# annikabrundyn/driving-dirty

Measured on AMD Instinct MI355X. Metric: 6-view scenes/sec fwd+bwd, roadmap model bs=32, higher is better.
Workload: dtype f32

## Files before the change

driving-dirty_amd/csrc/conv3x3.hip:

```cpp
#include <stdlib.h>

#include "dd_common.h"

namespace {

constexpr int EPI_BIAS_RELU_BITS = 5;
constexpr int EPI_RELU_BITS = 6;
constexpr int EPI_BIAS_STATS = 7;
constexpr int EPI_RELU_MASK_AFF = 8;
constexpr int EPI_RELU_BITS_W1 = 9;


template <int CIN, int S>
struct StripCfg {
  static constexpr int PXB = CIN * 4;
  static constexpr int CHUNKS = CIN / 4;
  static constexpr int NPX = 32 * S + 2;
  static constexpr int SLOTB = NPX * PXB;
  static constexpr int NCH = NPX * CHUNKS;
  static constexpr int NLOAD = (NCH + 63) / 64;
  static constexpr int SPILLB = (NLOAD * 64 - NCH) * 16;
  static constexpr int WAVEB = 3 * SLOTB + SPILLB;
  static constexpr int KGROUPS = (CIN == 32) ? 36 : 5;
  static constexpr int WFLOATS = KGROUPS * 64 * 4;
};

template <int CIN>
__device__ __forceinline__ int swz(int q) {
  return CIN == 32 ? ((q >> 1) & 7) : 0;
}

template <int CIN, int S>
__device__ __forceinline__ void load_row(const float* __restrict__ img, int H, int W, int iy, int gx0, int lane,
                                         f32x4 (&r)[StripCfg<CIN, S>::NLOAD]) {
  using C = StripCfg<CIN, S>;
  const bool rowok = (iy >= 0) && (iy < H);
  const __amdgpu_buffer_rsrc_t rs = dd_rsrc(img + (long)(rowok ? iy : 0) * W * CIN, rowok ? W * C::PXB : 0);
#pragma unroll
  for (int i = 0; i < C::NLOAD; ++i) {
    const int c = lane + 64 * i;
    const int q = c / C::CHUNKS, ch = c % C::CHUNKS;
    const int off = (c < C::NCH) ? ((gx0 + q) * C::PXB + ch * 16) : -16;
    r[i] = dd_bload4<DD_AUX_NT>(rs, off);
  }
}

template <int CIN, int S>
__device__ __forceinline__ void load_row_img(const float* __restrict__ img, int H, int W, int iy, int gx0, int lane,
                                             f32x4 (&r)[StripCfg<CIN, S>::NLOAD]) {
  using C = StripCfg<CIN, S>;
  const bool rowok = (iy >= 0) && (iy < H);
  const int so = rowok ? iy * W * C::PXB : 0;
  const __amdgpu_buffer_rsrc_t rs = dd_rsrc(img, rowok ? so + W * C::PXB : 0);
#pragma unroll
  for (int i = 0; i < C::NLOAD; ++i) {
    const int c = lane + 64 * i;
    const int q = c / C::CHUNKS, ch = c % C::CHUNKS;
    const int off = (c < C::NCH) ? ((gx0 + q) * C::PXB + ch * 16) : -16;
    r[i] = dd_bload4<DD_AUX_NT>(rs, off, so);
  }
}

template <int CIN, int S, bool SWZ>
__device__ __forceinline__ void store_row(char* slot, char* spill, int lane,
                                          const f32x4 (&r)[StripCfg<CIN, S>::NLOAD]) {
  using C = StripCfg<CIN, S>;
#pragma unroll
  for (int i = 0; i < C::NLOAD; ++i) {
    const int c = lane + 64 * i;
    const int q = c / C::CHUNKS, ch = c % C::CHUNKS;
    char* dst = slot + q * C::PXB + ((ch ^ (SWZ ? swz<CIN>(q) : 0)) << 4);
    if (64 * (i + 1) > C::NCH) dst = (c < C::NCH) ? dst : spill + (c - C::NCH) * 16;
    *(f32x4*)dst = r[i];
  }
}

template <int S, bool SWZ>
__device__ __forceinline__ void store_row_aff(char* slot, char* spill, int lane, const f32x4 (&r)[StripCfg<32, S>::NLOAD],
                                              bool rowok, int gx0, int W, f32x4 sc, f32x4 sh) {
  using C = StripCfg<32, S>;
#pragma unroll
  for (int i = 0; i < C::NLOAD; ++i) {
    const int c = lane + 64 * i;
    const int q = c / C::CHUNKS, ch = c % C::CHUNKS;
    char* dst = slot + q * C::PXB + ((ch ^ (SWZ ? swz<32>(q) : 0)) << 4);
    if (64 * (i + 1) > C::NCH) dst = (c < C::NCH) ? dst : spill + (c - C::NCH) * 16;
    const bool in = rowok && (gx0 + q >= 0) && (gx0 + q < W);
    f32x4 v = r[i];
    v.x = in ? fmaxf(v.x * sc.x + sh.x, 0.f) : 0.f;
    v.y = in ? fmaxf(v.y * sc.y + sh.y, 0.f) : 0.f;
    v.z = in ? fmaxf(v.z * sc.z + sh.z, 0.f) : 0.f;
    v.w = in ? fmaxf(v.w * sc.w + sh.w, 0.f) : 0.f;
    *(f32x4*)dst = v;
  }
}

template <int CIN, int S, int EPI, int WPB, bool AFF = false>
__global__ __launch_bounds__(WPB * 64) void conv_strip_fwd(const float* __restrict__ x, const float* __restrict__ wp,
                                                           const float* __restrict__ bias,
                                                           const float* __restrict__ msk, float* __restrict__ y,
                                                           unsigned* __restrict__ bits_out, int B, int H, int W, int Ho,
                                                           int Wo, int nstrips, const float* __restrict__ aff = nullptr,
                                                           float* __restrict__ stats = nullptr) {
  using C = StripCfg<CIN, S>;
  extern __shared__ __attribute__((aligned(16))) char smem[];
  const int tid = threadIdx.x;
  const int lane = tid & 63;
  const int wave = __builtin_amdgcn_readfirstlane(tid >> 6);
  {
    f32x4* wl4 = (f32x4*)smem;
    const f32x4* wg4 = (const f32x4*)wp;
    for (int i = tid; i < C::WFLOATS / 4; i += WPB * 64) wl4[i] = wg4[i];
  }
  __syncthreads();
  char* ring = smem + C::WFLOATS * 4 + wave * C::WAVEB;
  char* spill = ring + 3 * C::SLOTB;
  const char* wl = smem;
  const int h = lane >> 5, n = lane & 31;
  const float bv = (EPI == DD_EPI_BIAS || EPI == DD_EPI_BIAS_RELU || EPI == EPI_BIAS_RELU_BITS || EPI == EPI_BIAS_STATS) ? bias[n] : 0.f;
  f32x4 asc = {1.f, 1.f, 1.f, 1.f}, ash = {0.f, 0.f, 0.f, 0.f};
  if (AFF) {
    asc = *(const f32x4*)(aff + 4 * (lane & 7));
    ash = *(const f32x4*)(aff + 32 + 4 * (lane & 7));
  }
  const float msc = (EPI == EPI_RELU_MASK_AFF) ? aff[64 + n] : 1.f, msh = (EPI == EPI_RELU_MASK_AFF) ? aff[96 + n] : 0.f;
  float st_sum = 0.f, st_sq = 0.f;

  long idx, end;
  dd_range((long)B * nstrips * Ho, blockIdx.x * WPB + wave, gridDim.x * WPB, idx, end);
  while (idx < end) {
    const long col = idx / Ho;
    const int y0 = (int)(idx - col * Ho);
    const int y1 = (int)min((long)Ho, y0 + (end - idx));
    idx += y1 - y0;
    const int b = (int)(col / nstrips), x0 = (int)(col % nstrips) * 32;
    const float* xb = x + (long)b * H * W * CIN;
    const int gx0 = S * x0 - 1;

#pragma unroll
    for (int d = 0; d < 3; ++d) {
      f32x4 t[C::NLOAD];
      const int iy = S * y0 - 1 + d;
      load_row<CIN, S>(xb, H, W, iy, gx0, lane, t);
      if constexpr (AFF) store_row_aff<S, true>(ring + ((iy + 1) % 3) * C::SLOTB, spill, lane, t, iy >= 0 && iy < H, gx0, W, asc, ash);
      else store_row<CIN, S, true>(ring + ((iy + 1) % 3) * C::SLOTB, spill, lane, t);
    }

    for (int yy = y0; yy < y1; ++yy) {
      f32x4 pre[S][C::NLOAD];
#pragma unroll
      for (int s = 0; s < S; ++s) load_row<CIN, S>(xb, H, W, S * yy + 2 + s, gx0, lane, pre[s]);

      const long orow = ((long)(b * Ho + yy) * Wo) * 32;
      float mreg[16];
      if (EPI == DD_EPI_RELU_MASK || EPI == EPI_RELU_MASK_AFF) {
        const __amdgpu_buffer_rsrc_t ms = dd_rsrc(msk + orow, Wo * 128);
#pragma unroll
        for (int r = 0; r < 16; ++r) mreg[r] = dd_bload1<DD_AUX_NT>(ms, ((x0 + dd_acc_row(r, lane)) * 32 + n) * 4);
      }
      if (EPI == EPI_RELU_BITS) {
        const __amdgpu_buffer_rsrc_t ms = dd_rsrc((const unsigned*)msk + (long)(b * Ho + yy) * Wo, Wo * 4);
#pragma unroll
        for (int r = 0; r < 16; ++r) mreg[r] = dd_bload1<DD_AUX_NT>(ms, (x0 + dd_acc_row(r, lane)) * 4);
      }
      __builtin_amdgcn_sched_barrier(0);

      f32x16 acc;
#pragma unroll
      for (int r = 0; r < 16; ++r) acc[r] = 0.f;

      if (CIN == 32) {
#pragma unroll
        for (int dy = 0; dy < 3; ++dy) {
          const char* rowb = ring + ((S * yy + dy) % 3) * C::SLOTB;
#pragma unroll
          for (int dx = 0; dx < 3; ++dx) {
            const int q = S * n + dx;
            const char* pa = rowb + q * 128;
            const int sw = swz<32>(q);
#pragma unroll
            for (int j = 0; j < 4; ++j) {
              const f32x4 a = *(const f32x4*)(pa + (((2 * j + h) ^ sw) << 4));
              const f32x4 w = *(const f32x4*)(wl + (((dy * 3 + dx) * 4 + j) * 64 + lane) * 16);
              acc = DD_MFMA(a.x, w.x, acc);
              acc = DD_MFMA(a.y, w.y, acc);
              acc = DD_MFMA(a.z, w.z, acc);
              acc = DD_MFMA(a.w, w.w, acc);
            }
          }
        }
      } else {
#pragma unroll
        for (int jp = 0; jp < 5; ++jp) {
          const int tap = min(2 * jp + h, 8);
          const int dy = tap / 3, dx = tap - 3 * dy;
          const char* rowb = ring + ((S * yy + dy) % 3) * C::SLOTB;
          const f32x4 a = *(const f32x4*)(rowb + (S * n + dx) * 16);
          const f32x4 w = *(const f32x4*)(wl + (jp * 64 + lane) * 16);
          acc = DD_MFMA(a.x, w.x, acc);
          acc = DD_MFMA(a.y, w.y, acc);
          acc = DD_MFMA(a.z, w.z, acc);
        }
      }

#pragma unroll
      for (int s = 0; s < S; ++s) {
        const int iy = S * yy + 2 + s;
        if constexpr (AFF) store_row_aff<S, true>(ring + ((iy + 1) % 3) * C::SLOTB, spill, lane, pre[s], iy >= 0 && iy < H, gx0, W, asc, ash);
        else store_row<CIN, S, true>(ring + ((iy + 1) % 3) * C::SLOTB, spill, lane, pre[s]);
      }

      const __amdgpu_buffer_rsrc_t ys = dd_rsrc(y + orow, Wo * 128);
      unsigned sign_word = 0;
#pragma unroll
      for (int r = 0; r < 16; ++r) {
        float v = acc[r];
        if (EPI == DD_EPI_BIAS || EPI == EPI_BIAS_STATS) v += bv;
        if (EPI == EPI_BIAS_STATS && x0 + dd_acc_row(r, lane) < Wo) {
          st_sum += v;
          st_sq += v * v;
        }
        if (EPI == DD_EPI_BIAS_RELU || EPI == EPI_BIAS_RELU_BITS) v = fmaxf(v + bv, 0.f);
        if (EPI == DD_EPI_RELU_MASK) v = (mreg[r] > 0.f) ? v : 0.f;
        if (EPI == EPI_RELU_MASK_AFF) v = (mreg[r] * msc + msh > 0.f) ? v : 0.f;
        if (EPI == EPI_RELU_BITS) v = ((__builtin_bit_cast(unsigned, mreg[r]) >> n) & 1u) ? v : 0.f;
        dd_bstore1<DD_AUX_NT>(ys, ((x0 + dd_acc_row(r, lane)) * 32 + n) * 4, v);
        if (EPI == EPI_BIAS_RELU_BITS) {
          const unsigned long long m = __ballot(v > 0.f);
          const int i0 = (r & 3) + 8 * (r >> 2);
          if (n == i0) sign_word = (unsigned)m;
          if (n == i0 + 4) sign_word = (unsigned)(m >> 32);
        }
      }
      if (EPI == EPI_BIAS_RELU_BITS) {
        const __amdgpu_buffer_rsrc_t bs = dd_rsrc(bits_out + (long)(b * Ho + yy) * Wo, Wo * 4);
        __builtin_amdgcn_raw_buffer_store_b32(sign_word, bs, (h == 0) ? (x0 + n) * 4 : -16, 0, 0);
      }
    }
  }
  if (EPI == EPI_BIAS_STATS) {
    const long gwl = ((long)(blockIdx.x * WPB + wave) * 64 + lane) * 2;
    stats[gwl] = st_sum;
    stats[gwl + 1] = st_sq;
  }
}

template <int WPB, int MASK>
__global__ __launch_bounds__(WPB * 64) void conv_s2_dgrad(const float* __restrict__ dy, const float* __restrict__ wp,
                                                          const float* __restrict__ msk, float* __restrict__ dx,
                                                          int B, int H, int W, int Ho, int Wo, int nstrips,
                                                          const float* __restrict__ aff = nullptr) {
  using C = StripCfg<32, 1>;
  extern __shared__ __attribute__((aligned(16))) char smem[];
  const int tid = threadIdx.x;
  const int lane = tid & 63;
  const int wave = __builtin_amdgcn_readfirstlane(tid >> 6);
  {
    f32x4* wl4 = (f32x4*)smem;
    const f32x4* wg4 = (const f32x4*)wp;
    for (int i = tid; i < C::WFLOATS / 4; i += WPB * 64) wl4[i] = wg4[i];
  }
  __syncthreads();
  const int nr = (H + 1) / 2;
  const float msc = (MASK == 3) ? aff[64 + (lane & 31)] : 1.f, msh = (MASK == 3) ? aff[96 + (lane & 31)] : 0.f;
  char* ring = smem + C::WFLOATS * 4 + wave * C::WAVEB;
  char* spill = ring + 3 * C::SLOTB;
  const char* wl = smem;
  const int h = lane >> 5, n = lane & 31;

  long idx, end;
  dd_range((long)B * nstrips * nr, blockIdx.x * WPB + wave, gridDim.x * WPB, idx, end);
  while (idx < end) {
    const long col = idx / nr;
    const int r0 = (int)(idx - col * nr);
    const int r1 = (int)min((long)nr, r0 + (end - idx));
    idx += r1 - r0;
    const int b = (int)(col / nstrips), s0 = (int)(col % nstrips) * 32;
    const float* dyb = dy + (long)b * Ho * Wo * 32;

#pragma unroll
    for (int d = 0; d < 2; ++d) {
      f32x4 t[C::NLOAD];
      load_row<32, 1>(dyb, Ho, Wo, r0 + d, s0, lane, t);
      store_row<32, 1, true>(ring + ((r0 + d) % 3) * C::SLOTB, spill, lane, t);
    }

    for (int r = r0; r < r1; ++r) {
      f32x4 pre[C::NLOAD];
      load_row<32, 1>(dyb, Ho, Wo, r + 2, s0, lane, pre);
      __builtin_amdgcn_sched_barrier(0);

      const char* row_r = ring + (r % 3) * C::SLOTB;
      const char* row_r1 = ring + ((r + 1) % 3) * C::SLOTB;
#define DD_TILE(PY, PX, NTAP, ...)                                                              \
  {                                                                                             \
    constexpr int taps[NTAP][3] = {__VA_ARGS__};                                                \
    const int yi = 2 * r + (PY);                                                                \
    const long orow = ((long)(b * H + min(yi, H - 1)) * W) * 32;                                \
    const int obytes = (yi < H) ? W * 128 : 0;                                                  \
    float mreg[16];                                                                             \
    if (MASK == 1 || MASK == 3) {                                                               \
      const __amdgpu_buffer_rsrc_t ms = dd_rsrc(msk + orow, obytes);                            \
      _Pragma("unroll") for (int rr = 0; rr < 16; ++rr)                                         \
        mreg[rr] = dd_bload1<DD_AUX_NT>(ms, ((2 * (s0 + dd_acc_row(rr, lane)) + (PX)) * 32 + n) * 4); \
      __builtin_amdgcn_sched_barrier(0);                                                        \
    }                                                                                           \
    if (MASK == 2) {                                                                            \
      const __amdgpu_buffer_rsrc_t ms = dd_rsrc((const unsigned*)msk + (long)(b * H + min(yi, H - 1)) * W, obytes / 32); \
      _Pragma("unroll") for (int rr = 0; rr < 16; ++rr)                                         \
        mreg[rr] = dd_bload1<DD_AUX_NT>(ms, (2 * (s0 + dd_acc_row(rr, lane)) + (PX)) * 4);      \
      __builtin_amdgcn_sched_barrier(0);                                                        \
    }                                                                                           \
    f32x16 acc;                                                                                 \
    _Pragma("unroll") for (int i = 0; i < 16; ++i) acc[i] = 0.f;                                \
    _Pragma("unroll") for (int t = 0; t < NTAP; ++t) {                                          \
      const char* rowp = taps[t][0] ? row_r1 : row_r;                                           \
      const int q = n + taps[t][1];                                                             \
      const char* pa = rowp + q * 128;                                                          \
      const int sw = swz<32>(q);                                                                \
      _Pragma("unroll") for (int j = 0; j < 4; ++j) {                                           \
        const f32x4 a = *(const f32x4*)(pa + (((2 * j + h) ^ sw) << 4));                        \
        const f32x4 w = *(const f32x4*)(wl + ((taps[t][2] * 4 + j) * 64 + lane) * 16);          \
        acc = DD_MFMA(a.x, w.x, acc);                                                           \
        acc = DD_MFMA(a.y, w.y, acc);                                                           \
        acc = DD_MFMA(a.z, w.z, acc);                                                           \
        acc = DD_MFMA(a.w, w.w, acc);                                                           \
      }                                                                                         \
    }                                                                                           \
    const __amdgpu_buffer_rsrc_t os = dd_rsrc(dx + orow, obytes);                               \
    _Pragma("unroll") for (int rr = 0; rr < 16; ++rr) {                                         \
      float v = acc[rr];                                                                        \
      if (MASK == 1) v = (mreg[rr] > 0.f) ? v : 0.f;                                            \
      if (MASK == 3) v = (mreg[rr] * msc + msh > 0.f) ? v : 0.f;                                \
      if (MASK == 2) v = ((__builtin_bit_cast(unsigned, mreg[rr]) >> n) & 1u) ? v : 0.f;        \
      dd_bstore1<DD_AUX_NT>(os, ((2 * (s0 + dd_acc_row(rr, lane)) + (PX)) * 32 + n) * 4, v);    \
    }                                                                                           \
  }
      DD_TILE(1, 1, 4, {1, 1, 0}, {1, 0, 2}, {0, 1, 6}, {0, 0, 8})
      store_row<32, 1, true>(ring + ((r + 2) % 3) * C::SLOTB, spill, lane, pre);
      DD_TILE(0, 1, 2, {0, 1, 3}, {0, 0, 5})
      DD_TILE(1, 0, 2, {1, 0, 1}, {0, 0, 7})
      DD_TILE(0, 0, 1, {0, 0, 4})
#undef DD_TILE
    }
  }
}

template <int CIN, int S, int WPB, bool AFF = false>
__global__ __launch_bounds__(WPB * 64) void conv_wgrad(const float* __restrict__ x, const float* __restrict__ dy,
                                                       float* __restrict__ part, float* __restrict__ bpart, int B,
                                                       int H, int W, int Ho, int Wo, int nstrips,
                                                       const float* __restrict__ aff = nullptr) {
  using C = StripCfg<CIN, S>;
  constexpr int NT = (CIN == 32) ? 9 : 1;
  extern __shared__ __attribute__((aligned(16))) char smem[];
  const int tid = threadIdx.x;
  const int lane = tid & 63;
  const int wave = __builtin_amdgcn_readfirstlane(tid >> 6);
  char* ring = smem + wave * C::WAVEB;
  char* spill = ring + 3 * C::SLOTB;
  const int h = lane >> 5, n = lane & 31;
  const int gw = blockIdx.x * WPB + wave;
  f32x4 asc = {1.f, 1.f, 1.f, 1.f}, ash = {0.f, 0.f, 0.f, 0.f};
  if (AFF) {
    asc = *(const f32x4*)(aff + 4 * (lane & 7));
    ash = *(const f32x4*)(aff + 32 + 4 * (lane & 7));
  }

  f32x16 acc[NT];
#pragma unroll
  for (int t = 0; t < NT; ++t)
#pragma unroll
    for (int r = 0; r < 16; ++r) acc[t][r] = 0.f;
  float bsum = 0.f;

  const int tap4 = min(n / 3, 8), c4 = n % 3;
  const int dy4 = tap4 / 3, dx4 = tap4 - 3 * dy4;

  long idx, end;
  dd_range((long)B * nstrips * Ho, gw, gridDim.x * WPB, idx, end);
  while (idx < end) {
    const long col = idx / Ho;
    const int y0 = (int)(idx - col * Ho);
    const int y1 = (int)min((long)Ho, y0 + (end - idx));
    idx += y1 - y0;
    const int b = (int)(col / nstrips), x0 = (int)(col % nstrips) * 32;
    const float* xb = x + (long)b * H * W * CIN;
    const float* dyb = dy + (long)b * Ho * Wo * 32;
    const int gx0 = S * x0 - 1;
    const int aoff = ((x0 + h) * 32 + n) * 4;

#pragma unroll
    for (int d = 0; d < 3; ++d) {
      f32x4 t[C::NLOAD];
      const int iy = S * y0 - 1 + d;
      load_row<CIN, S>(xb, H, W, iy, gx0, lane, t);
      if constexpr (AFF) store_row_aff<S, false>(ring + ((iy + 1) % 3) * C::SLOTB, spill, lane, t, iy >= 0 && iy < H, gx0, W, asc, ash);
      else store_row<CIN, S, false>(ring + ((iy + 1) % 3) * C::SLOTB, spill, lane, t);
    }
    float areg[16];
    {
      const __amdgpu_buffer_rsrc_t as = dd_rsrc(dyb + (long)y0 * Wo * 32, Wo * 128);
#pragma unroll
      for (int pp = 0; pp < 16; ++pp) areg[pp] = dd_bload1<DD_AUX_NT>(as, aoff + pp * 256);
    }

    for (int yy = y0; yy < y1; ++yy) {
      f32x4 pre[S][C::NLOAD];
#pragma unroll
      for (int s = 0; s < S; ++s) load_row<CIN, S>(xb, H, W, S * yy + 2 + s, gx0, lane, pre[s]);
      float anext[16];
      {
        const bool ok = yy + 1 < Ho;
        const __amdgpu_buffer_rsrc_t as = dd_rsrc(dyb + (long)(ok ? yy + 1 : 0) * Wo * 32, ok ? Wo * 128 : 0);
#pragma unroll
        for (int pp = 0; pp < 16; ++pp) anext[pp] = dd_bload1<DD_AUX_NT>(as, aoff + pp * 256);
      }
      __builtin_amdgcn_sched_barrier(0);

      if (CIN == 32) {
        const char* rb0 = ring + ((S * yy + 0) % 3) * C::SLOTB;
        const char* rb1 = ring + ((S * yy + 1) % 3) * C::SLOTB;
        const char* rb2 = ring + ((S * yy + 2) % 3) * C::SLOTB;
#pragma unroll
        for (int pp = 0; pp < 16; ++pp) {
          const float a = areg[pp];
          bsum += a;
          const int off = (S * (2 * pp + h)) * 128 + n * 4;
#pragma unroll
          for (int dx = 0; dx < 3; ++dx) {
            acc[0 + dx] = DD_MFMA(a, *(const float*)(rb0 + off + dx * 128), acc[0 + dx]);
            acc[3 + dx] = DD_MFMA(a, *(const float*)(rb1 + off + dx * 128), acc[3 + dx]);
            acc[6 + dx] = DD_MFMA(a, *(const float*)(rb2 + off + dx * 128), acc[6 + dx]);
          }
        }
      } else {
        const char* rb = ring + ((S * yy + dy4) % 3) * C::SLOTB + dx4 * 16 + c4 * 4;
#pragma unroll
        for (int pp = 0; pp < 16; ++pp) {
          const float a = areg[pp];
          bsum += a;
          acc[0] = DD_MFMA(a, *(const float*)(rb + (S * (2 * pp + h)) * 16), acc[0]);
        }
      }

#pragma unroll
      for (int s = 0; s < S; ++s) {
        const int iy = S * yy + 2 + s;
        if constexpr (AFF) store_row_aff<S, false>(ring + ((iy + 1) % 3) * C::SLOTB, spill, lane, pre[s], iy >= 0 && iy < H, gx0, W, asc, ash);
        else store_row<CIN, S, false>(ring + ((iy + 1) % 3) * C::SLOTB, spill, lane, pre[s]);
      }
#pragma unroll
      for (int pp = 0; pp < 16; ++pp) areg[pp] = anext[pp];
    }
  }

#pragma unroll
  for (int t = 0; t < NT; ++t)
#pragma unroll
    for (int r = 0; r < 16; ++r) part[(((long)gw * NT + t) * 16 + r) * 64 + lane] = acc[t][r];
  bpart[(long)gw * 64 + lane] = bsum;
}

template <int CIN>
__global__ __launch_bounds__(1024) void conv_wgrad_reduce(const float* __restrict__ part,
                                                          const float* __restrict__ bpart, float* __restrict__ dw,
                                                          float* __restrict__ db, int nw) {
  constexpr int NT = (CIN == 32) ? 9 : 1;
  constexpr int G = 16;
  __shared__ double red[G][64];
  const int l = threadIdx.x & 63, g = threadIdx.x >> 6;
  const int row = blockIdx.x;
  const float* src = (row < NT * 16) ? part + (long)row * 64 + l : bpart + l;
  const long stride = (row < NT * 16) ? (long)NT * 16 * 64 : 64;
  double s0 = 0.0, s1 = 0.0, s2 = 0.0, s3 = 0.0;
  int w = g;
  for (; w + 3 * G < nw; w += 4 * G) {
    s0 += (double)src[(long)w * stride];
    s1 += (double)src[(long)(w + G) * stride];
    s2 += (double)src[(long)(w + 2 * G) * stride];
    s3 += (double)src[(long)(w + 3 * G) * stride];
  }
  for (; w < nw; w += G) s0 += (double)src[(long)w * stride];
  red[g][l] = (s0 + s1) + (s2 + s3);
  __syncthreads();
  if (g != 0) return;
  double sd = 0.0;
#pragma unroll
  for (int i = 0; i < G; ++i) sd += red[i][l];
  const float s = (float)sd;
  if (row < NT * 16) {
    const int t = row >> 4, r = row & 15;
    const int o = dd_acc_row(r, l), j = l & 31;
    if (CIN == 32) {
      dw[((long)o * 32 + j) * 9 + t] = s;
    } else if (j < 27) {
      dw[((long)o * 3 + (j % 3)) * 9 + (j / 3)] = s;
    }
  } else {
    const double other = __shfl_xor(sd, 32);
    if (l < 32) db[l] = (float)(sd + other);
  }
}

__global__ void conv_pack_kernel(const float* __restrict__ w, float* __restrict__ p, int cin_real, int kind) {
  const int idx = blockIdx.x * blockDim.x + threadIdx.x;
  if (cin_real == 32) {
    if (idx >= 36 * 64 * 4) return;
    const int i = idx & 3, lane = (idx >> 2) & 63, g = idx >> 8;
    const int j = g & 3, t = g >> 2;
    const int n = lane & 31, c = 8 * j + 4 * (lane >> 5) + i;
    float v;
    if (kind == 0) v = w[((long)n * 32 + c) * 9 + t];
    else if (kind == 1) v = w[((long)c * 32 + n) * 9 + (8 - t)];
    else v = w[((long)c * 32 + n) * 9 + t];
    p[idx] = v;
  } else {
    if (idx >= 5 * 64 * 4) return;
    const int i = idx & 3, lane = (idx >> 2) & 63, jp = idx >> 8;
    const int n = lane & 31, tap = 2 * jp + (lane >> 5);
    p[idx] = (tap < 9 && i < 3) ? w[((long)n * 3 + i) * 9 + tap] : 0.f;
  }
}

constexpr int WINO_UFLOATS = 3 * 4 * 2 * 2 * 64 * 4;

__device__ __forceinline__ f32x2 pk_sub2(f32x2 a, f32x2 b) {
  f32x2 r;
  asm("v_pk_add_f32 %0, %1, %2 neg_lo:[0,1] neg_hi:[0,1]" : "=v"(r) : "v"(a), "v"(b));
  return r;
}
__device__ __forceinline__ f32x2 pk_add2(f32x2 a, f32x2 b) {
  f32x2 r;
  asm("v_pk_add_f32 %0, %1, %2" : "=v"(r) : "v"(a), "v"(b));
  return r;
}
__device__ __forceinline__ f32x4 pk_add4a(f32x4 a, f32x4 b) {
  const f32x2 lo = pk_add2(f32x2{a.x, a.y}, f32x2{b.x, b.y}), hi = pk_add2(f32x2{a.z, a.w}, f32x2{b.z, b.w});
  return f32x4{lo.x, lo.y, hi.x, hi.y};
}
__device__ __forceinline__ f32x4 pk_add4(f32x4 a, f32x4 b) {
  const f32x2 lo = f32x2{a.x, a.y} + f32x2{b.x, b.y}, hi = f32x2{a.z, a.w} + f32x2{b.z, b.w};
  return f32x4{lo.x, lo.y, hi.x, hi.y};
}
__device__ __forceinline__ f32x4 pk_sub4(f32x4 a, f32x4 b) {
  f32x2 lo, hi;
  const f32x2 alo = {a.x, a.y}, ahi = {a.z, a.w}, blo = {b.x, b.y}, bhi = {b.z, b.w};
  asm("v_pk_add_f32 %0, %1, %2 neg_lo:[0,1] neg_hi:[0,1]" : "=v"(lo) : "v"(alo), "v"(blo));
  asm("v_pk_add_f32 %0, %1, %2 neg_lo:[0,1] neg_hi:[0,1]" : "=v"(hi) : "v"(ahi), "v"(bhi));
  return f32x4{lo.x, lo.y, hi.x, hi.y};
}

template <int EPI, int WPB>
__global__ __launch_bounds__(WPB * 64) void conv_wino_fwd(const float* __restrict__ x, const float* __restrict__ up,
                                                          const float* __restrict__ bias, const unsigned* __restrict__ bits_in,
                                                          float* __restrict__ y, unsigned* __restrict__ bits_out, int B, int H,
                                                          int W, int nstrips) {
  using C = StripCfg<32, 1>;
  extern __shared__ __attribute__((aligned(16))) char smem[];
  const int tid = threadIdx.x;
  const int lane = tid & 63;
  const int wave = __builtin_amdgcn_readfirstlane(tid >> 6);
  {
    f32x4* ul4 = (f32x4*)smem;
    const f32x4* ug4 = (const f32x4*)up;
    for (int i = tid; i < WINO_UFLOATS / 4; i += WPB * 64) ul4[i] = ug4[i];
  }
  __syncthreads();
  char* ring = smem + WINO_UFLOATS * 4 + wave * C::WAVEB;
  char* spill = ring + 3 * C::SLOTB;
  const f32x4* ul = (const f32x4*)smem;
  const int t16 = lane & 15, q4 = lane >> 4;
  const float bv0 = (EPI == EPI_BIAS_RELU_BITS) ? bias[t16] : 0.f, bv1 = (EPI == EPI_BIAS_RELU_BITS) ? bias[16 + t16] : 0.f;

  long idx, end;
  dd_range((long)B * nstrips * H, blockIdx.x * WPB + wave, gridDim.x * WPB, idx, end);
  while (idx < end) {
    const long col = idx / H;
    const int y0 = (int)(idx - col * H);
    const int y1 = (int)min((long)H, y0 + (end - idx));
    idx += y1 - y0;
    const int b = (int)(col / nstrips), x0 = (int)(col % nstrips) * 32;
    const float* xb = x + (long)b * H * W * 32;
    const int gx0 = x0 - 1;

#pragma unroll
    for (int d = 0; d < 3; ++d) {
      f32x4 t[C::NLOAD];
      const int iy = y0 - 1 + d;
      load_row<32, 1>(xb, H, W, iy, gx0, lane, t);
      store_row<32, 1, true>(ring + ((iy + 1) % 3) * C::SLOTB, spill, lane, t);
    }

    for (int yy = y0; yy < y1; ++yy) {
      f32x4 pre[C::NLOAD];
      load_row<32, 1>(xb, H, W, yy + 2, gx0, lane, pre);
      const long opix = (long)(b * H + yy) * W;
      unsigned mw[8];
      if (EPI == EPI_RELU_BITS) {
        const __amdgpu_buffer_rsrc_t ms = dd_rsrc(bits_in + opix, W * 4);
#pragma unroll
        for (int i = 0; i < 8; ++i)
          mw[i] = __builtin_amdgcn_raw_buffer_load_b32(ms, (x0 + 8 * q4 + i) * 4, 0, 0);
      }
      __builtin_amdgcn_sched_barrier(0);

      f32x4 acc[4][2];
#pragma unroll
      for (int p = 0; p < 4; ++p)
#pragma unroll
        for (int hf = 0; hf < 2; ++hf) acc[p][hf] = f32x4{0.f, 0.f, 0.f, 0.f};

      f32x4 dbuf[2][4], ubuf[2][4][2];
      auto rd = [&](int it, f32x4 (&d)[4], f32x4 (&u)[4][2]) {
        const int ky = it >> 1, g = it & 1;
        const char* rowb = ring + ((yy + ky) % 3) * C::SLOTB;
#pragma unroll
        for (int c = 0; c < 4; ++c) {
          const int px = 2 * t16 + c;
          d[c] = *(const f32x4*)(rowb + px * 128 + (((2 * q4 + g) ^ swz<32>(px)) << 4));
        }
#pragma unroll
        for (int p = 0; p < 4; ++p)
#pragma unroll
          for (int hf = 0; hf < 2; ++hf) u[p][hf] = ul[((((ky * 4 + p) * 2 + hf) * 2 + g) * 64) + lane];
      };
      f32x4 vbuf[2][4];
      auto tf = [&](const f32x4 (&d)[4], f32x4 (&v)[4]) {
        v[0] = pk_sub4(d[0], d[2]);
        v[1] = pk_add4(d[1], d[2]);
        v[2] = pk_sub4(d[2], d[1]);
        v[3] = pk_sub4(d[1], d[3]);
      };
      rd(0, dbuf[0], ubuf[0]);
      tf(dbuf[0], vbuf[0]);
#pragma unroll
      for (int it = 0; it < 6; ++it) {
        if (it + 1 < 6) {
          rd(it + 1, dbuf[(it + 1) & 1], ubuf[(it + 1) & 1]);
          tf(dbuf[(it + 1) & 1], vbuf[(it + 1) & 1]);
        }
        __builtin_amdgcn_sched_barrier(0);
        const f32x4(&u)[4][2] = ubuf[it & 1];
        const f32x4(&v)[4] = vbuf[it & 1];
#pragma unroll
        for (int j = 0; j < 4; ++j)
#pragma unroll
          for (int p = 0; p < 4; ++p)
#pragma unroll
            for (int hf = 0; hf < 2; ++hf) acc[p][hf] = DD_MFMA16(v[p][j], u[p][hf][j], acc[p][hf]);
        __builtin_amdgcn_sched_barrier(0);
      }

      store_row<32, 1, true>(ring + ((yy + 3) % 3) * C::SLOTB, spill, lane, pre);

      const __amdgpu_buffer_rsrc_t ys = dd_rsrc(y + opix * 32, W * 128);
      unsigned keep[8];
#pragma unroll
      for (int i = 0; i < 8; ++i) keep[i] = 0;
#pragma unroll
      for (int r = 0; r < 4; ++r) {
#pragma unroll
        for (int e = 0; e < 2; ++e) {
          const int opx = x0 + 2 * (4 * q4 + r) + e;
          float o[2];
#pragma unroll
          for (int hf = 0; hf < 2; ++hf) {
            const float m0 = acc[0][hf][r], m1 = acc[1][hf][r], m2 = acc[2][hf][r], m3 = acc[3][hf][r];
            float v = e == 0 ? (m0 + m1) + m2 : (m1 - m2) - m3;
            if (EPI == EPI_BIAS_RELU_BITS) v = fmaxf(v + (hf ? bv1 : bv0), 0.f);
            if (EPI == EPI_RELU_BITS) {
              v = ((mw[2 * r + e] >> (t16 + 16 * hf)) & 1u) ? v : 0.f;
            }
            o[hf] = v;
            dd_bstore1<DD_AUX_NT>(ys, (opx * 32 + t16 + 16 * hf) * 4, v);
          }
          if (EPI == EPI_BIAS_RELU_BITS) {
            const unsigned long long b0 = __ballot(o[0] > 0.f), b1 = __ballot(o[1] > 0.f);
            const int G = (lane & 31) >> 3;
            const unsigned w = (unsigned)((b0 >> (16 * G)) & 0xffffull) | ((unsigned)((b1 >> (16 * G)) & 0xffffull) << 16);
            keep[2 * r + e] = w;
          }
        }
      }
      if (EPI == EPI_BIAS_RELU_BITS) {
        const int P = lane & 31, sel = P & 7;
        unsigned word = keep[0];
#pragma unroll
        for (int i = 1; i < 8; ++i) word = (sel == i) ? keep[i] : word;
        const __amdgpu_buffer_rsrc_t bs = dd_rsrc(bits_out + opix, W * 4);
        __builtin_amdgcn_raw_buffer_store_b32(word, bs, (lane < 32) ? (x0 + P) * 4 : -16, 0, 0);
      }
    }
  }
}

constexpr int WINO2_UFLOATS = 16 * 2 * 2 * 64 * 4;

template <int EPI, int WPB>
__global__ __launch_bounds__(WPB * 64) void conv_wino2_fwd(const float* __restrict__ x, const float* __restrict__ up,
                                                           const float* __restrict__ bias, const unsigned* __restrict__ bits_in,
                                                           float* __restrict__ y, unsigned* __restrict__ bits_out, int B, int H,
                                                           int W, int nstrips, const float* __restrict__ x4 = nullptr,
                                                           float* __restrict__ w1part = nullptr) {
  using C = StripCfg<32, 1>;
  using C4 = StripCfg<4, 1>;
  constexpr int RINGB = 4 * C::SLOTB + C::SPILLB;
  constexpr bool W1 = (EPI == EPI_RELU_BITS_W1);
  constexpr bool MASKED = (EPI == EPI_RELU_BITS) || W1;
  extern __shared__ __attribute__((aligned(16))) char smem[];
  const int tid = threadIdx.x;
  const int lane = tid & 63;
  const int wave = __builtin_amdgcn_readfirstlane(tid >> 6);
  {
    f32x4* ul4 = (f32x4*)smem;
    const f32x4* ug4 = (const f32x4*)up;
    for (int i = tid; i < WINO2_UFLOATS / 4; i += WPB * 64) ul4[i] = ug4[i];
  }
  constexpr int W2_XRINGB = 4 * C4::SLOTB + C4::SPILLB;
  constexpr int W2_XBASE = WINO2_UFLOATS * 4 + WPB * RINGB;
  if (W1 && tid < 32) ((float*)(smem + W2_XBASE + WPB * W2_XRINGB))[tid] = 1.f;
  __syncthreads();
  char* xring = smem + W2_XBASE + wave * W2_XRINGB;
  char* xspill = xring + 4 * C4::SLOTB;
  f32x4 wacc[2][2];
#pragma unroll
  for (int hf = 0; hf < 2; ++hf)
#pragma unroll
    for (int nh = 0; nh < 2; ++nh) wacc[hf][nh] = f32x4{0.f, 0.f, 0.f, 0.f};
  char* ring = smem + WINO2_UFLOATS * 4 + wave * RINGB;
  char* spill = ring + 4 * C::SLOTB;
  const f32x4* ul = (const f32x4*)smem;
  const int t16 = lane & 15, q4 = lane >> 4;
  int xky[2], xlane[2];
#pragma unroll
  for (int nh = 0; nh < 2; ++nh) {
    const int c = min(t16 + 16 * nh, 26), tap = c / 3, ci = c - 3 * tap, ky = tap / 3, kx = tap - 3 * ky;
    xky[nh] = ky;
    xlane[nh] = (8 * q4 + kx) * 16 + ci * 4;
  }
  const float bv0 = (EPI == EPI_BIAS_RELU_BITS) ? bias[t16] : 0.f, bv1 = (EPI == EPI_BIAS_RELU_BITS) ? bias[16 + t16] : 0.f;
  const f32x4 bias0 = {bv0, bv0, bv0, bv0}, bias1 = {bv1, bv1, bv1, bv1};
  const int HT = (H + 1) / 2;

  long idx, end;
  dd_range((long)B * nstrips * HT, blockIdx.x * WPB + wave, gridDim.x * WPB, idx, end);
  while (idx < end) {
    const long col = idx / HT;
    const int r0 = (int)(idx - col * HT);
    const int r1 = (int)min((long)HT, r0 + (end - idx));
    idx += r1 - r0;
    const int b = (int)(col / nstrips), x0 = (int)(col % nstrips) * 32;
    const float* xb = x + (long)b * H * W * 32;
// ... 1590 lines not shown
```

Measured before the change: 4353.

## Software-pipeline transposed-conv dgrad and wgrad loops with interleaved LDS, MFMA and stores

Restructures the stride-2 transposed conv backward-data loop so LDS operand reads are double-buffered one group ahead. The previous tile's output stores, the next tile's mask loads and the ring-buffer row writes are interleaved between MFMAs using sched_group_barrier. The wgrad CIN=32 path likewise prefetches ring reads one step ahead and spreads the ring writes of the next rows into the MFMA stream. The aim is to hide LDS and global memory latency behind matrix math instead of running them in separate phases. This adds register pressure from the mreg[4][16] and pend buffers, and ordering constraints that rely on static_asserts about when ring slots are last read.

```diff
diff --git a/driving-dirty_amd/csrc/conv3x3.hip b/driving-dirty_amd/csrc/conv3x3.hip
--- a/driving-dirty_amd/csrc/conv3x3.hip
+++ b/driving-dirty_amd/csrc/conv3x3.hip
@@ -94,6 +94,30 @@
     *(f32x4*)dst = v;
   }
 }
+
+template <int CIN, int S, bool SWZ>
+__device__ __forceinline__ char* ring_chunk(char* slot, char* spill, int lane, int i) {
+  using C = StripCfg<CIN, S>;
+  const int c = lane + 64 * i;
+  const int q = c / C::CHUNKS, ch = c % C::CHUNKS;
+  char* dst = slot + q * C::PXB + ((ch ^ (SWZ ? swz<CIN>(q) : 0)) << 4);
+  if (64 * (i + 1) > C::NCH) dst = (c < C::NCH) ? dst : spill + (c - C::NCH) * 16;
+  return dst;
+}
+template <int S>
+__device__ __forceinline__ f32x4 aff_chunk(f32x4 v, int lane, int i, bool rowok, int gx0, int W, f32x4 sc, f32x4 sh) {
+  const int q = (lane + 64 * i) / StripCfg<32, S>::CHUNKS;
+  const bool in = rowok && (gx0 + q >= 0) && (gx0 + q < W);
+  v.x = in ? fmaxf(v.x * sc.x + sh.x, 0.f) : 0.f;
+  v.y = in ? fmaxf(v.y * sc.y + sh.y, 0.f) : 0.f;
+  v.z = in ? fmaxf(v.z * sc.z + sh.z, 0.f) : 0.f;
+  v.w = in ? fmaxf(v.w * sc.w + sh.w, 0.f) : 0.f;
+  return v;
+}
+template <bool V>
+struct BoolTag {
+  static constexpr bool value = V;
+};
 
 template <int CIN, int S, int EPI, int WPB, bool AFF = false>
 __global__ __launch_bounds__(WPB * 64) void conv_strip_fwd(const float* __restrict__ x, const float* __restrict__ wp,
@@ -285,64 +309,105 @@
       store_row<32, 1, true>(ring + ((r0 + d) % 3) * C::SLOTB, spill, lane, t);
     }
 
-    for (int r = r0; r < r1; ++r) {
+    constexpr int taps[9][3] = {{1, 1, 0}, {1, 0, 2}, {0, 1, 6}, {0, 0, 8},
+                                {0, 1, 3}, {0, 0, 5},
+                                {1, 0, 1}, {0, 0, 7},
+                                {0, 0, 4}};
+    constexpr int first[5] = {0, 16, 24, 32, 36};
+    float mreg[4][16], pend[16];
+    f32x16 acc;
+    f32x4 a[2], w[2];
+
+    const int pix0 = 2 * (s0 + 4 * h);
+    const int soff0 = (pix0 * 32 + n) * 4, moff0 = pix0 * 4;
+    auto mask_load = [&](int rr, int k, int i) {
+      const int yi = 2 * rr + (k == 0 || k == 2), pc = 2 * ((i & 3) + 8 * (i >> 2)) + (k < 2);
+      const int obytes = (yi < H) ? W * 128 : 0;
+      if (MASK == 1 || MASK == 3) {
+        const __amdgpu_buffer_rsrc_t ms = dd_rsrc(msk + ((long)(b * H + min(yi, H - 1)) * W) * 32, obytes);
+        mreg[k][i] = dd_bload1<DD_AUX_NT>(ms, soff0, pc * 128);
+      }
+      if (MASK == 2) {
+        const __amdgpu_buffer_rsrc_t ms = dd_rsrc((const unsigned*)msk + (long)(b * H + min(yi, H - 1)) * W, obytes / 32);
+        mreg[k][i] = dd_bload1<DD_AUX_NT>(ms, moff0, pc * 4);
+      }
+    };
+    auto tile_store = [&](int rr, int k, int i) {
+      const int yi = 2 * rr + (k == 0 || k == 2), pc = 2 * ((i & 3) + 8 * (i >> 2)) + (k < 2);
+      const __amdgpu_buffer_rsrc_t os = dd_rsrc(dx + ((long)(b * H + min(yi, H - 1)) * W) * 32, (yi < H) ? W * 128 : 0);
+      dd_bstore<DD_AUX_NT>(os, soff0, pend[i], pc * 128);
+    };
+    auto rd = [&](int rr, int g, f32x4& av, f32x4& wv) {
+      const int t = g >> 2, j = g & 3;
+      const int q = n + taps[t][1];
+      av = *(const f32x4*)(ring + ((rr + taps[t][0]) % 3) * C::SLOTB + q * 128 + (((2 * j + h) ^ swz<32>(q)) << 4));
+      wv = *(const f32x4*)(wl + ((taps[t][2] * 4 + j) * 64 + lane) * 16);
+    };
+    auto pair = [&](auto first_tag, int r) {
+      constexpr bool FIRST = decltype(first_tag)::value;
       f32x4 pre[C::NLOAD];
       load_row<32, 1>(dyb, Ho, Wo, r + 2, s0, lane, pre);
       __builtin_amdgcn_sched_barrier(0);
-
-      const char* row_r = ring + (r % 3) * C::SLOTB;
-      const char* row_r1 = ring + ((r + 1) % 3) * C::SLOTB;
-#define DD_TILE(PY, PX, NTAP, ...)                                                              \
-  {                                                                                             \
-    constexpr int taps[NTAP][3] = {__VA_ARGS__};                                                \
-    const int yi = 2 * r + (PY);                                                                \
-    const long orow = ((long)(b * H + min(yi, H - 1)) * W) * 32;                                \
-    const int obytes = (yi < H) ? W * 128 : 0;                                                  \
-    float mreg[16];                                                                             \
-    if (MASK == 1 || MASK == 3) {                                                               \
-      const __amdgpu_buffer_rsrc_t ms = dd_rsrc(msk + orow, obytes);                            \
-      _Pragma("unroll") for (int rr = 0; rr < 16; ++rr)                                         \
-        mreg[rr] = dd_bload1<DD_AUX_NT>(ms, ((2 * (s0 + dd_acc_row(rr, lane)) + (PX)) * 32 + n) * 4); \
-      __builtin_amdgcn_sched_barrier(0);                                                        \
-    }                                                                                           \
-    if (MASK == 2) {                                                                            \
-      const __amdgpu_buffer_rsrc_t ms = dd_rsrc((const unsigned*)msk + (long)(b * H + min(yi, H - 1)) * W, obytes / 32); \
-      _Pragma("unroll") for (int rr = 0; rr < 16; ++rr)                                         \
-        mreg[rr] = dd_bload1<DD_AUX_NT>(ms, (2 * (s0 + dd_acc_row(rr, lane)) + (PX)) * 4);      \
-      __builtin_amdgcn_sched_barrier(0);                                                        \
-    }                                                                                           \
-    f32x16 acc;                                                                                 \
-    _Pragma("unroll") for (int i = 0; i < 16; ++i) acc[i] = 0.f;                                \
-    _Pragma("unroll") for (int t = 0; t < NTAP; ++t) {                                          \
-      const char* rowp = taps[t][0] ? row_r1 : row_r;                                           \
-      const int q = n + taps[t][1];                                                             \
-      const char* pa = rowp + q * 128;                                                          \
-      const int sw = swz<32>(q);                                                                \
-      _Pragma("unroll") for (int j = 0; j < 4; ++j) {                                           \
-        const f32x4 a = *(const f32x4*)(pa + (((2 * j + h) ^ sw) << 4));                        \
-        const f32x4 w = *(const f32x4*)(wl + ((taps[t][2] * 4 + j) * 64 + lane) * 16);          \
-        acc = DD_MFMA(a.x, w.x, acc);                                                           \
-        acc = DD_MFMA(a.y, w.y, acc);                                                           \
-        acc = DD_MFMA(a.z, w.z, acc);                                                           \
-        acc = DD_MFMA(a.w, w.w, acc);                                                           \
-      }                                                                                         \
-    }                                                                                           \
-    const __amdgpu_buffer_rsrc_t os = dd_rsrc(dx + orow, obytes);                               \
-    _Pragma("unroll") for (int rr = 0; rr < 16; ++rr) {                                         \
-      float v = acc[rr];                                                                        \
-      if (MASK == 1) v = (mreg[rr] > 0.f) ? v : 0.f;                                            \
-      if (MASK == 3) v = (mreg[rr] * msc + msh > 0.f) ? v : 0.f;                                \
-      if (MASK == 2) v = ((__builtin_bit_cast(unsigned, mreg[rr]) >> n) & 1u) ? v : 0.f;        \
-      dd_bstore1<DD_AUX_NT>(os, ((2 * (s0 + dd_acc_row(rr, lane)) + (PX)) * 32 + n) * 4, v);    \
-    }                                                                                           \
-  }
-      DD_TILE(1, 1, 4, {1, 1, 0}, {1, 0, 2}, {0, 1, 6}, {0, 0, 8})
-      store_row<32, 1, true>(ring + ((r + 2) % 3) * C::SLOTB, spill, lane, pre);
-      DD_TILE(0, 1, 2, {0, 1, 3}, {0, 0, 5})
-      DD_TILE(1, 0, 2, {1, 0, 1}, {0, 0, 7})
-      DD_TILE(0, 0, 1, {0, 0, 4})
-#undef DD_TILE
-    }
+#pragma unroll
+      for (int k = 0; k < 4; ++k) {
+        constexpr int NG[4] = {16, 8, 8, 4};
+        const int g0 = first[k], per = 16 / NG[k];
+#pragma unroll
+        for (int i = 0; i < 16; ++i) acc[i] = 0.f;
+#pragma unroll
+        for (int g = g0; g < g0 + NG[k]; ++g) {
+          __builtin_amdgcn_sched_barrier(0);
+          if (g + 1 < 36) rd(r, g + 1, a[(g + 1) & 1], w[(g + 1) & 1]);
+          else rd(r + 1, 0, a[0], w[0]);
+#pragma unroll
+          for (int e = 0; e < 4; ++e) {
+            acc = DD_MFMA(a[g & 1][e], w[g & 1][e], acc);
+            if (e < per) {
+              const int i = (g - g0) * per + e;
+              if (!(FIRST && k == 0)) tile_store(k == 0 ? r - 1 : r, (k + 3) & 3, i);
+              if (MASK != 0) mask_load(k >= 2 ? r + 1 : r, (k + 2) & 3, i);
+            }
+            if (e == 0 && k == 2 && g - g0 < C::NLOAD)
+              *(f32x4*)ring_chunk<32, 1, true>(ring + ((r + 2) % 3) * C::SLOTB, spill, lane, g - g0) = pre[g - g0];
+          }
+          __builtin_amdgcn_sched_group_barrier(0x100, 2, 0);
+#pragma unroll
+          for (int e = 0; e < 4; ++e) {
+            __builtin_amdgcn_sched_group_barrier(0x008, 1, 0);
+            if (e < per) {
+              __builtin_amdgcn_sched_group_barrier(0x040, 1, 0);
+              __builtin_amdgcn_sched_group_barrier(0x020, 1, 0);
+            }
+            if (e == 0) __builtin_amdgcn_sched_group_barrier(0x200, 1, 0);
+          }
+        }
+        __builtin_amdgcn_sched_barrier(0);
+#pragma unroll
+        for (int i = 0; i < 16; ++i) {
+          float v = acc[i];
+          if (MASK == 1) v = (mreg[k][i] > 0.f) ? v : 0.f;
+          if (MASK == 3) v = (mreg[k][i] * msc + msh > 0.f) ? v : 0.f;
+          if (MASK == 2)
+            v = __builtin_bit_cast(float, __builtin_bit_cast(int, v) & __builtin_amdgcn_sbfe(__builtin_bit_cast(int, mreg[k][i]), (unsigned)n, 1u));
+          pend[i] = v;
+        }
+        __builtin_amdgcn_sched_barrier(0);
+      }
+    };
+
+    static_assert(C::NLOAD <= 8, "the ring writes of a row go behind the 8 groups of tile 2");
+    if (MASK != 0) {
+#pragma unroll
+      for (int i = 0; i < 16; ++i) {
+        mask_load(r0, 0, i);
+        mask_load(r0, 1, i);
+      }
+    }
+    rd(r0, 0, a[0], w[0]);
+    pair(BoolTag<true>{}, r0);
+    for (int r = r0 + 1; r < r1; ++r) pair(BoolTag<false>{}, r);
+#pragma unroll
+    for (int i = 0; i < 16; ++i) tile_store(r1 - 1, 3, i);
   }
 }
 
@@ -418,22 +483,40 @@
       }
       __builtin_amdgcn_sched_barrier(0);
 
-      if (CIN == 32) {
-        const char* rb0 = ring + ((S * yy + 0) % 3) * C::SLOTB;
-        const char* rb1 = ring + ((S * yy + 1) % 3) * C::SLOTB;
-        const char* rb2 = ring + ((S * yy + 2) % 3) * C::SLOTB;
-#pragma unroll
-        for (int pp = 0; pp < 16; ++pp) {
-          const float a = areg[pp];
-          bsum += a;
-          const int off = (S * (2 * pp + h)) * 128 + n * 4;
-#pragma unroll
-          for (int dx = 0; dx < 3; ++dx) {
-            acc[0 + dx] = DD_MFMA(a, *(const float*)(rb0 + off + dx * 128), acc[0 + dx]);
-            acc[3 + dx] = DD_MFMA(a, *(const float*)(rb1 + off + dx * 128), acc[3 + dx]);
-            acc[6 + dx] = DD_MFMA(a, *(const float*)(rb2 + off + dx * 128), acc[6 + dx]);
+      if constexpr (CIN == 32) {
+#pragma unroll
+        for (int pp = 0; pp < 16; ++pp) bsum += areg[pp];
+        __builtin_amdgcn_sched_barrier(0);
+        constexpr int NW = S * C::NLOAD, GW = 48 - NW;
+        static_assert(GW >= 15 && GW + (S - 1) * C::NLOAD >= 16 * (S - 1) + 15, "ring write before the slot's last reader");
+        float bq[2][3];
+        auto rd = [&](int st, float (&v)[3]) {
+          const int k = st >> 4, pp = st & 15;
+          const char* rb = ring + ((S * yy + k) % 3) * C::SLOTB + (S * (2 * pp + h)) * 128 + n * 4;
+#pragma unroll
+          for (int dx = 0; dx < 3; ++dx) v[dx] = *(const float*)(rb + dx * 128);
+        };
+        rd(0, bq[0]);
+#pragma unroll
+        for (int st = 0; st < 48; ++st) {
+          __builtin_amdgcn_sched_barrier(0);
+          if (st + 1 < 48) rd(st + 1, bq[(st + 1) & 1]);
+          const int k = st >> 4, pp = st & 15;
+          acc[3 * k + 0] = DD_MFMA(areg[pp], bq[st & 1][0], acc[3 * k + 0]);
+          if (st >= GW) {
+            const int s = (st - GW) / C::NLOAD, i = (st - GW) % C::NLOAD, iy = S * yy + 2 + s;
+            char* dst = ring_chunk<CIN, S, false>(ring + ((iy + 1) % 3) * C::SLOTB, spill, lane, i);
+            if constexpr (AFF) *(f32x4*)dst = aff_chunk<S>(pre[s][i], lane, i, iy >= 0 && iy < H, gx0, W, asc, ash);
+            else *(f32x4*)dst = pre[s][i];
           }
-        }
+          acc[3 * k + 1] = DD_MFMA(areg[pp], bq[st & 1][1], acc[3 * k + 1]);
+          acc[3 * k + 2] = DD_MFMA(areg[pp], bq[st & 1][2], acc[3 * k + 2]);
+          __builtin_amdgcn_sched_group_barrier(0x100, 3, 0);
+          __builtin_amdgcn_sched_group_barrier(0x008, 1, 0);
+          __builtin_amdgcn_sched_group_barrier(0x200, 1, 0);
+          __builtin_amdgcn_sched_group_barrier(0x008, 2, 0);
+        }
+        __builtin_amdgcn_sched_barrier(0);
       } else {
         const char* rb = ring + ((S * yy + dy4) % 3) * C::SLOTB + dx4 * 16 + c4 * 4;
 #pragma unroll
@@ -442,13 +525,8 @@
           bsum += a;
           acc[0] = DD_MFMA(a, *(const float*)(rb + (S * (2 * pp + h)) * 16), acc[0]);
         }
-      }
-
-#pragma unroll
-      for (int s = 0; s < S; ++s) {
-        const int iy = S * yy + 2 + s;
-        if constexpr (AFF) store_row_aff<S, false>(ring + ((iy + 1) % 3) * C::SLOTB, spill, lane, pre[s], iy >= 0 && iy < H, gx0, W, asc, ash);
-        else store_row<CIN, S, false>(ring + ((iy + 1) % 3) * C::SLOTB, spill, lane, pre[s]);
+#pragma unroll
+        for (int s = 0; s < S; ++s) store_row<CIN, S, false>(ring + ((S * yy + 2 + s + 1) % 3) * C::SLOTB, spill, lane, pre[s]);
       }
 #pragma unroll
       for (int pp = 0; pp < 16; ++pp) areg[pp] = anext[pp];
```

New measurement: 4382 (median of 6 runs). Within noise of the previous version (+0.7%).
